# mpkuse/cerebro

Hardware: AMD Instinct MI355X
Metric: loop-queries/sec (ticks of 3 descriptors vs 4096-D x 1M DB) (higher is better)
Workload: dtype f64

## Files before the change

cerebro_amd/csrc/chip_api.hip:

```cpp
#include "chip_internal.h"
#include <cmath>
#include <cstdlib>
#include <cstring>
#include <memory>
#include <new>

using namespace chip;

extern "C" {

const char *chip_strerror(int status)
{
    switch (status) {
        case CHIP_OK: return "ok";
        case CHIP_ERR_INVALID_ARG: return "invalid argument";
        case CHIP_ERR_NO_DEVICE: return "no usable HIP device";
        case CHIP_ERR_HIP: return "HIP runtime error (see chip_last_hip_error)";
        case CHIP_ERR_OOM: return "out of device memory";
        case CHIP_ERR_NOT_F32: return "descriptor value not exactly representable as float32";
        case CHIP_ERR_NONFINITE: return "NaN/Inf in descriptor";
        case CHIP_ERR_RANGE: return "index / length out of range";
        case CHIP_ERR_UNSUPPORTED: return "unsupported configuration";
        case CHIP_ERR_TOO_FEW_POINTS: return "fewer than 20 correspondences";
        case CHIP_ERR_BUSY: return "async slot busy or empty";
// ... 178 lines not shown
    int rc = c->seg_table_dev.alloc(c, kMaxSegs);
    if (rc == CHIP_OK) rc = configure_storage(c, elem);
    if (rc != CHIP_OK) return rc;
    c->stage_bytes = 64ull << 20;
    if (c->stage_bytes < (size_t)c->D * 8 * 64) c->stage_bytes = (size_t)c->D * 8 * 64;
    rc = c->stage_dev.alloc(c, c->stage_bytes);
    if (rc == CHIP_OK) rc = c->flags_dev.alloc(c, 1);
    if (rc == CHIP_OK) rc = c->flags_host.alloc(c, 1);
    if (rc == CHIP_OK) rc = c->norm2_dev.alloc(c, 1);
    if (rc == CHIP_OK) rc = c->norm2_host.alloc(c, 1);
    if (rc != CHIP_OK) return rc;
    CHIP_HIP(c, hipMemset(c->norm2_dev, 0, sizeof(unsigned long long)));
    *c->norm2_host.host() = 0;

    scan_read_knobs(c);
    CHIP_HIP(c, hipStreamCreateWithFlags(&c->s_scan, hipStreamNonBlocking));
    {
        const int ns = c->scan_streams;
        if (ns >= 2) CHIP_HIP(c, hipStreamCreateWithFlags(&c->s_scan2, hipStreamNonBlocking));
        for (int i = 0; i < 2; i++)
            if (ns >= 3 + i) CHIP_HIP(c, hipStreamCreateWithFlags(&c->s_scan_x[i], hipStreamNonBlocking));
    }
    for (int i = 0; i < Ctx::kRing; i++) {
        constexpr size_t kListsPerGroup = 3 * kPrefilterTicks > CHIP_MAX_NQ ? 3 * kPrefilterTicks : CHIP_MAX_NQ;
        static_assert(kPrefilterTicks >= kMultiMaxTicks, "the list buffers are sized for the deepest pass");
        rc = c->partial_dev[i].alloc(c, ((size_t)c->max_grid + 1) * kListsPerGroup * CHIP_MAX_TOPK);
        if (rc != CHIP_OK) return rc;
        CHIP_HIP(c, hipEventCreateWithFlags(&c->ev_scan[i], hipEventDisableTiming));
        CHIP_HIP(c, hipEventCreateWithFlags(&c->ev_merged[i], hipEventDisableTiming));
    }
    rc = c->tickets_dev.alloc(c, Ctx::kRing);
    if (rc != CHIP_OK) return rc;
    CHIP_HIP(c, hipMemset(c->tickets_dev, 0, Ctx::kRing * sizeof(int32_t)));
    c->coalesce_max = env_int("CHIP_TICK_COALESCE", kPrefilterTicks);
    if (c->coalesce_max < 2) c->coalesce_max = 0;
    if (c->coalesce_max > kPrefilterTicks) c->coalesce_max = kPrefilterTicks;
    c->tick_poll = env_int("CHIP_TICK_POLL", 1) != 0;
    resident_read_knobs(c);
    rc = c->seq_all.alloc(c, CHIP_MAX_INFLIGHT);
    if (rc != CHIP_OK) return rc;
    std::memset(c->seq_all.host(), 0, sizeof(unsigned long long) * CHIP_MAX_INFLIGHT);
    rc = c->cert_all.alloc(c, CHIP_MAX_INFLIGHT * 4);
    if (rc != CHIP_OK) return rc;
    std::memset(c->cert_all.host(), 0, sizeof(uint32_t) * CHIP_MAX_INFLIGHT * 4);
    rc = c->topk.alloc(c, (size_t)CHIP_MAX_NQ * CHIP_MAX_TOPK);
    if (rc != CHIP_OK) return rc;
    for (Slot &s : c->slots) {
        CHIP_HIP(c, hipEventCreateWithFlags(&s.done, hipEventDisableTiming));
        rc = s.rec.alloc(c, 1);
        if (rc != CHIP_OK) return rc;
        s.seq_host = c->seq_all.host() + (&s - c->slots);
        s.seq_dev = c->seq_all.dev() + (&s - c->slots);
        s.cert_host = c->cert_all.host() + 4 * (&s - c->slots);
        s.cert_dev = c->cert_all.dev() + 4 * (&s - c->slots);
    }
    if (env_int("CHIP_SCAN_STAMPS", 0)) {
        rc = c->stamps_dev.alloc(c, (size_t)c->max_grid * 16 * 4 + 64);
        if (rc != CHIP_OK) return rc;
        CHIP_HIP(c, hipMemset(c->stamps_dev, 0, ((size_t)c->max_grid * 16 * 4 + 64) * sizeof(unsigned long long)));
    }
    rc = pnp_create(c);
    if (rc != CHIP_OK) return rc;
    c->cap_hint = capacity_hint;
    if (capacity_hint > 0) {
        std::lock_guard<std::mutex> lk(c->append_mu);
        rc = ensure_capacity(c, local_count(c, capacity_hint));
// ... 260 lines not shown
    int fit = scan_multi_max_ticks(c);
    if (c->coalesce_max >= kPrefilterTicks && scan_prefilter_usable(c)) fit = kPrefilterTicks;
    const int t = fit < c->coalesce_max ? fit : c->coalesce_max;
    return t >= 2 ? t : 0;
}

static int coalesce_submit(Ctx *c, int T)
{
    const int b = (int)(c->n_enqueued++ % Ctx::kRing);
    const int K = CHIP_DEFAULT_TOPK;
    const bool prefilter = T == kPrefilterTicks;
    static_assert(kPrefilterTicks > kMultiMaxTicks, "a pass of kPrefilterTicks ticks is the prefilter's");
    PassArgs a{};
    scan_args_db(c, &a);
    a.K = K;
    a.partial = c->partial_dev[b];
    for (int t = 0; t < T; t++) {
        a.k[t] = c->parked[t].k;
        if (a.k[t] > a.n_rows) a.n_rows = a.k[t];
        for (int i = 0; i < 3; i++) a.q[3 * t + i] = c->parked[t].q[i];
    }
    const int grid = scan_multi_grid(c);
    double E = 0.0;
    if (prefilter) {
        std::lock_guard<std::mutex> lk(c->mu);
        E = prefilter_error_bound(c->D, c->row_norm_max);
    }
    if (hipEventQuery(c->ev_merged[b]) != hipSuccess) CHIP_HIP(c, hipStreamWaitEvent(c->s_scan, c->ev_merged[b], 0));
    hipEvent_t e1 = nullptr;
    int rc = c->prof_on ? prof_begin(c, c->s_scan, (double)a.n_rows * c->D * c->elem, &e1) : CHIP_OK;
    if (rc == CHIP_OK) rc = prefilter ? launch_scan_prefilter(c, c->s_scan, a, grid) : launch_scan_multi(c, c->s_scan, a, T, grid);
    if (rc != CHIP_OK) return rc;
    if (e1) CHIP_HIP(c, hipEventRecord(e1, c->s_scan));
    CHIP_HIP(c, hipEventRecord(c->ev_scan[b], c->s_scan));
    c->pass_ev = c->ev_scan[b];
    c->pass_no++;
    CHIP_HIP(c, hipStreamWaitEvent(c->s_query, c->ev_scan[b], 0));
    chip_topk_entry *exact = c->partial_dev[b] + (size_t)kPrefilterTicks * grid * 3 * K;
    if (prefilter) {
        RescoreArgs ra{};
        ra.seg_table = a.seg_table; ra.seg_shift = a.seg_shift; ra.seg_mask = a.seg_mask; ra.D = a.D; ra.K = K;
        ra.in = c->partial_dev[b]; ra.n_lists = grid; ra.wpb = 8;
        ra.E = E;
        ra.out = exact;
        for (int t = 0; t < T; t++) {
            const Ctx::ParkedTick &pt = c->parked[t];
            Slot &s = *pt.slot;
            ra.k[t] = pt.k;
            for (int i = 0; i < 3; i++) { ra.q[3 * t + i] = s.pf_q[i] = pt.q[i]; s.cert_host[i] = 0; }
            ra.cert[t] = s.cert_dev;
            s.prefilter = true; s.pf_k = pt.k; s.pf_p = pt.p;
        }
        rc = launch_rescore(c, c->s_query, ra);
        if (rc != CHIP_OK) return rc;
    }
    for (int t = 0; t < T; t++) {
        const Ctx::ParkedTick &pt = c->parked[t];
        if (prefilter) rc = launch_merge(c, c->s_query, merge_args(exact + (size_t)t * 3 * K, 1, K, nullptr, pt.slot->rec.dev(), pt.l, &pt.p), 3);
        else rc = launch_merge(c, c->s_query, merge_args(c->partial_dev[b] + (size_t)t * grid * 3 * K, grid, K, nullptr, pt.slot->rec.dev(), pt.l, &pt.p), 3);
        if (rc != CHIP_OK) return rc;
        CHIP_HIP(c, hipEventRecord(pt.slot->done, c->s_query));
        pt.slot->wait_ev = pt.slot->done;
        pt.slot->state = SlotState::Event;
        pt.slot->pass_no = c->pass_no;
    }
    CHIP_HIP(c, hipEventRecord(c->ev_merged[b], c->s_query));
    c->coalesce_passes++;
    c->coalesce_ticks += T;
    if (prefilter) { c->prefilter_passes++; c->prefilter_ticks += T; }
    return CHIP_OK;
}

int coalesce_flush(Ctx *c)
{
    const int T = c->n_parked;
    if (T == 0) return CHIP_OK;
    c->n_parked = 0;
    const Ctx::ParkedTick &p0 = c->parked[0];
    int rc;
    if (T == kPrefilterTicks && !scan_prefilter_usable(c)) {
        const Ctx::ParkedTick &pl = c->parked[T - 1];
        rc = coalesce_submit(c, T - 1);
        if (rc == CHIP_OK) rc = tick_submit(c, pl.k, pl.l, &pl.p, pl.q, false, *pl.slot);
    } else {
        rc = T == 1 ? tick_submit(c, p0.k, p0.l, &p0.p, p0.q, false, *p0.slot) : coalesce_submit(c, T);
    }
    for (int t = 0; t < T && rc != CHIP_OK; t++) {
        c->parked[t].slot->state = SlotState::Failed;
        c->parked[t].slot->err = rc;
    }
    return rc;
}

static int tick_enqueue_slot(Ctx *c, int64_t l, const chip_dot_params *p, bool sync_tick, Slot &s)
{
    int32_t status = 0;
    int64_t k = 0;
    const int64_t n_pub = published_rows(c);
    int rc = tick_begin(s, c->xchg ? INT64_MAX : n_pub, &c->last_l, l, p, &status, &k);
// ... 871 lines not shown
```

cerebro_amd/csrc/chip_internal.h:

```cpp
#pragma once
#include <hip/hip_runtime.h>
#include <cstdint>
#include <mutex>
#include <utility>
#include <condition_variable>
#include <vector>
#include "../../include/cerebro_hip.h"

namespace chip {

constexpr int kWave = 64;
constexpr int kMaxSegs = 4096;
constexpr int64_t kSegBytesTarget = 512ll << 20;

struct ScanArgs {
    const void *const *seg_table;
    int32_t seg_shift;
    int64_t seg_mask;
    int64_t n_rows;
    int32_t D;
    int32_t K;
    const void *q[CHIP_MAX_NQ];
    int64_t idx_mul, idx_add;
    chip_topk_entry *partial;
// ... 33 lines not shown
    unsigned long long *exit_host;
    unsigned long long instance;
    unsigned long long lease_ticks;
    uint32_t done;
    uint32_t direct;
};

constexpr int kMultiMaxTicks = 3;
constexpr int kPrefilterTicks = 4;
constexpr int kRescoreCap = 32;
struct PassArgs {
    const void *const *seg_table;
    int32_t seg_shift;
    int64_t seg_mask;
    int64_t n_rows;
    int32_t D;
    int32_t K;
    int64_t k[kPrefilterTicks];
    const void *q[3 * kPrefilterTicks];
    chip_topk_entry *partial;
};
struct RescoreArgs {
    const void *const *seg_table;
    int32_t seg_shift;
    int64_t seg_mask;
    int32_t D;
    int32_t K;
    const chip_topk_entry *in;
    int32_t n_lists;
    int32_t wpb;
    int64_t k[kPrefilterTicks];
    const void *q[3 * kPrefilterTicks];
    double E;
    chip_topk_entry *out;
    uint32_t *cert[kPrefilterTicks];
};

struct MergeArgs {
    const chip_topk_entry *in;
    int32_t n_lists;
    int32_t K;
    chip_topk_entry *out;
    chip_tick_result *result;
    int64_t l;
    int32_t locality;
    double thresh;
};

struct Ctx;

template <class T> class DevBuf {
public:
    DevBuf() = default;
    DevBuf(const DevBuf &) = delete;
    DevBuf &operator=(const DevBuf &) = delete;
    ~DevBuf() { release(); }
    int alloc(Ctx *c, size_t n);
    int reserve(Ctx *c, size_t n);
    void release() { if (p_) (void)hipFree(p_); p_ = nullptr; cap_ = 0; }
    void swap(DevBuf &o) { std::swap(p_, o.p_); std::swap(cap_, o.cap_); }
    T *get() const { return p_; }
    operator T *() const { return p_; }
    size_t capacity() const { return cap_; }
private:
    T *p_ = nullptr;
    size_t cap_ = 0;
};
template <class T> class PinnedBuf {
// ... 38 lines not shown
int project_chunk(Ctx *c, int64_t from, int64_t m);
void project_count_reset(Ctx *c);

struct Vlad {
    DevBuf<char> w;
    DevBuf<float> raw;
    DevBuf<float> x;
    DevBuf<double> a;
    DevBuf<double> part;
    DevBuf<double> vu;
    DevBuf<float> out;
    int32_t C = 0, K = 0, G = 0;
    int32_t last_n = 0;
    int32_t last_maps = 0;
    int bias_count() const { return (K + G + 1) & ~1; }
    double *bias() const { return reinterpret_cast<double *>(w.get()); }
    float *Wt() const { return reinterpret_cast<float *>(w.get() + (size_t)bias_count() * sizeof(double)); }
    float *centres() const { return Wt() + (size_t)(K + G) * C; }
};
int vlad_chunk(Ctx *c, const AppendSrc &src, int64_t from, int64_t m);

int launch_resident(Ctx *c, hipStream_t s, const ResidentArgs &ra, int grid);
int launch_scan(Ctx *c, hipStream_t s, const ScanArgs &a, int nq, int grid);
int launch_merge(Ctx *c, hipStream_t s, const MergeArgs &a, int nq);
int scan_multi_max_ticks(const Ctx *c);
int scan_multi_plan(int D, int elem, int n_ticks, int K, int grid, chip_debug_scan_launch *f);
int scan_multi_grid(const Ctx *c);
int launch_scan_multi(Ctx *c, hipStream_t s, const PassArgs &a, int n_ticks, int grid);
int scan_prefilter_plan(int D, int elem, int K, int grid, chip_debug_scan_launch *f);
bool scan_prefilter_usable(const Ctx *c);
double prefilter_error_bound(int D, double row_norm_max);
int launch_scan_prefilter(Ctx *c, hipStream_t s, const PassArgs &a, int grid);
int launch_rescore(Ctx *c, hipStream_t s, const RescoreArgs &a);
int scan_grid_for(const Ctx *c, int64_t n_rows, int nq, bool q64);
bool scan_q64(const Ctx *c, int nq, bool long_scan);
int scan_rows_form(const Ctx *c, int64_t n_rows, int nq, int grid, bool q64, bool sync_tick = false);
int scan_select(const Ctx *c, const ScanArgs &a, int nq, int grid, chip_debug_scan_launch *f);
int scan_forms_built();
int launch_scores(Ctx *c, hipStream_t s, const ScanArgs &a, double *out_dev);
int launch_store_rows(Ctx *c, hipStream_t s, const void *src, int src_elem, int64_t n, int64_t first_global, uint32_t *flags_dev, bool write_ring,
                      int64_t row_stride = 1);
int launch_synth(Ctx *c, hipStream_t s, int64_t first_global, int64_t n, uint64_t seed,
                 const int64_t *plant_dst_dev, const int64_t *plant_src_dev, const int32_t *plant_kind_dev, int64_t n_plant, int unit);

enum class SlotState : uint8_t {
    Free,
    Immediate,
    Parked,
    Event,
    Poll,
    Resident,
    Failed,
};

struct Slot {
    hipEvent_t done = nullptr;
    hipEvent_t wait_ev = nullptr;
    PinnedBuf<chip_tick_result> rec;
    SlotState state = SlotState::Free;
    int64_t prev_last_l = 0;
    int64_t tick_l = 0;
    unsigned long long *seq_host = nullptr, *seq_dev = nullptr;
    unsigned long long seq_want = 0;
    uint64_t pass_no = 0;
    int32_t err = 0;
    bool prefilter = false;
// ... 61 lines not shown
    int64_t rows_global = 0;
    int64_t rows_local = 0;
    int64_t lossy_rows = 0;
    mutable std::mutex mu;
    std::mutex append_mu;
    mutable std::mutex query_mu;
    std::mutex ring_mu;
    int64_t rows_pending = 0;
    hipEvent_t last_scan_ev[2] = {};
    std::mutex pnp_mu;
    std::mutex icp_mu;

    hipStream_t s_query = nullptr, s_append = nullptr, s_pnp = nullptr;
    bool own_query_stream = true;

    DevBuf<char> stage_dev;
    size_t stage_bytes = 0;
    DevBuf<uint32_t> flags_dev;
    PinnedBuf<uint32_t> flags_host;
    DevBuf<unsigned long long> norm2_dev;
    PinnedBuf<unsigned long long> norm2_host;
    double row_norm_max = 0.0;

    static constexpr int kRing = 64;
    hipStream_t s_scan = nullptr;
    hipStream_t s_scan2 = nullptr;
    hipStream_t s_scan_x[2] = {};
    uint64_t n_same_stream = 0;
    DevBuf<chip_topk_entry> partial_dev[kRing];
    int32_t partial_lists[kRing] = {};
    hipEvent_t ev_scan[kRing] = {};
    hipEvent_t ev_merged[kRing] = {};
    DevBuf<int32_t> tickets_dev;
    PinnedBuf<unsigned long long> seq_all;
    unsigned long long tick_seq = 0;
    bool tick_poll = true;
    bool tick_fused = true;
    Resident res;
    uint64_t n_enqueued = 0;
    int32_t max_grid = 0;
    PinnedBuf<chip_topk_entry> topk;

    DevBuf<char> qvec_dev;
    DevBuf<double> scores_dev;
    DevBuf<unsigned long long> stamps_dev;

    std::vector<char> qconv;
    int64_t cap_hint = 0;
    int32_t group_transport = 0;
    mutable int last_comm = 0;
    int32_t comm_init_abandoned = 0;
    Exchange *xchg = nullptr;
    Group *group = nullptr;
    Ctx *parent = nullptr;
    Slot slots[CHIP_MAX_INFLIGHT];
    int64_t last_l = 0;

    struct ParkedTick { Slot *slot; int64_t k, l; chip_dot_params p; const void *q[3]; };
    int32_t coalesce_max = 4;
    bool coalesce_force = false;
    ParkedTick parked[kPrefilterTicks];
    int32_t n_parked = 0;
    hipEvent_t pass_ev = nullptr;
    uint64_t pass_no = 0;
    int64_t coalesce_passes = 0, coalesce_ticks = 0;
    int64_t prefilter_passes = 0, prefilter_ticks = 0, prefilter_uncertified = 0;
// ... 231 lines not shown
```

cerebro_amd/csrc/kernels.hip:

```cpp
#include "chip_internal.h"
#include "topk_merge.h"
#include <cmath>
#include <type_traits>

namespace chip {

typedef float f32x4 __attribute__((ext_vector_type(4)));
typedef double f64x2 __attribute__((ext_vector_type(2)));

template <typename T> struct Vec16;
template <> struct Vec16<float> { typedef f32x4 type; static constexpr int N = 4; };
template <> struct Vec16<double> { typedef f64x2 type; static constexpr int N = 2; };

template <typename V>
__device__ __forceinline__ const __attribute__((address_space(1))) V *as_global(const V *p)
{
    return (const __attribute__((address_space(1))) V *)p;
}

template <typename V>
__device__ __forceinline__ V stream_load(const V *p)
{
    return __builtin_nontemporal_load(as_global(p));
}
// ... 607 lines not shown
        constexpr int SS = U * NS;
        f32x4 w[SS];
        w[0] = *reinterpret_cast<const f32x4 *>(qv);
        w[1] = *reinterpret_cast<const f32x4 *>(qv + D);
        static_for<U>([&](auto uc) CHIP_INLINE_LAMBDA {
            constexpr int u = uc;
            slot_wait<L - R>();
            static_for<NS>([&](auto qc) CHIP_INLINE_LAMBDA {
                constexpr int q = qc, i = u * NS + q;
                if constexpr (i + 2 < SS) w[i + 2] = *reinterpret_cast<const f32x4 *>(qv + ((i + 2) % NS) * D + ((i + 2) / NS) * 256);
                const f32x2 wl = __builtin_shufflevector(w[i], w[i], 0, 1), wh = __builtin_shufflevector(w[i], w[i], 2, 3);
                static_for<R>([&](auto rr) CHIP_INLINE_LAMBDA { prefilter_fma<pass_row_slot(u, rr)>(acc[rr][q], wl); });
                static_for<R>([&](auto rr) CHIP_INLINE_LAMBDA { prefilter_fma<pass_row_slot(u, rr) + 2>(acc[rr][q], wh); });
                __builtin_amdgcn_sched_barrier(0);
            });
            static_for<NG>([&](auto gc) CHIP_INLINE_LAMBDA {
                constexpr int g = gc, QR = pass_query_slot(NG, u, g);
                slot_wait<L - R - 1 - g>();
                static_for<R>([&](auto rr) CHIP_INLINE_LAMBDA { prefilter_fma_slot<pass_row_slot(u, rr), QR>(acc[rr][NS + g]); });
                static_for<R>([&](auto rr) CHIP_INLINE_LAMBDA { prefilter_fma_slot<pass_row_slot(u, rr) + 2, QR + 2>(acc[rr][NS + g]); });
            });
            slots_issue_kib<u, NG>(voff, row, qg);
        });
    }
};

template <int NG>
__global__ __launch_bounds__(kMultiBlock) __attribute__((amdgpu_num_vgpr(pass_vgpr_base(kPrefilterMaxNG) / 2))) void db_scan_prefilter(PassArgs a)
{
    static_assert(NG <= kPrefilterMaxNG, "the compiler's share is sized for kPrefilterMaxNG query slots per KiB");
    shared_pass<PassF32<NG>>(a);
}

__device__ __forceinline__ void block_best(double &bs, int64_t &bi, double *red_s, int64_t *red_i, int lane, int wave)
{
#pragma unroll
    for (int m = 32; m >= 1; m >>= 1) {
        const double os = __shfl_xor(bs, m, 64);
        const int64_t oi = __shfl_xor(bi, m, 64);
        if (key_gt(os, oi, bs, bi)) { bs = os; bi = oi; }
    }
    __syncthreads();
    if (lane == 0) { red_s[wave] = bs; red_i[wave] = bi; }
    __syncthreads();
    bs = red_s[0]; bi = red_i[0];
#pragma unroll
    for (int w = 1; w < 8; w++)
        if (key_gt(red_s[w], red_i[w], bs, bi)) { bs = red_s[w]; bi = red_i[w]; }
}

__global__ __launch_bounds__(512) void tick_rescore(RescoreArgs a)
{
    constexpr int MAXH = 512 * CHIP_MAX_TOPK / 512;
    __shared__ double red_s[8];
    __shared__ int64_t red_i[8];
    __shared__ chip_topk_entry cand[kRescoreCap];
    __shared__ int n_cand;
    const int tid = threadIdx.x, lane = tid & 63;
    const int wave = __builtin_amdgcn_readfirstlane(tid >> 6);
    const int tick = blockIdx.x / 3, q = blockIdx.x % 3;
    const int K = a.K, n = a.n_lists * K;
    const chip_topk_entry *in = a.in + (int64_t)tick * a.n_lists * 3 * K;
    const int64_t k = a.k[tick];
    if (tid == 0) n_cand = 0;
    double es[MAXH];
    int64_t ei[MAXH];
// ... 17 lines not shown
    block_best(ms, mi, red_s, red_i, lane, wave);
    double gs = INFINITY;
    int64_t gi = INT64_MAX;
    for (int j = 0; j < K; j++) {
        double bs = -INFINITY;
        int64_t bi = -1;
#pragma unroll
        for (int h = 0; h < MAXH; h++)
            if (key_gt(gs, gi, es[h], ei[h]) && key_gt(es[h], ei[h], bs, bi)) { bs = es[h]; bi = ei[h]; }
        block_best(bs, bi, red_s, red_i, lane, wave);
        gs = bs; gi = bi;
    }
    double thr = gs - 2.0 * a.E;
    thr -= fabs(thr) * 0x1p-51;
    const bool ok = mi < 0 || ms < thr;
#pragma unroll
    for (int h = 0; h < MAXH; h++)
        if (ei[h] >= 0 && es[h] >= thr) {
            const int at = atomicAdd(&n_cand, 1);
            if (at < kRescoreCap) { chip_topk_entry t; t.score = es[h]; t.idx = ei[h]; cand[at] = t; }
        }
    __syncthreads();
    const int nc = n_cand < kRescoreCap ? n_cand : kRescoreCap;
    const float *qrow = static_cast<const float *>(a.q[3 * tick + q]);
    for (int j = wave; j < nc; j += 8) {
        const int64_t r = cand[j].idx;
        const float *row[1] = {static_cast<const float *>(a.seg_table[r >> a.seg_shift]) + (r & a.seg_mask) * (int64_t)a.D};
        double acc[1][1];
        rows_dot<float, 1, 4, true, 1, 1>(row, qrow, a.D, lane, acc);
        const double s = butterfly_sum(acc[0][0]);
        if (lane == 0) cand[j].score = s;
    }
    __syncthreads();
    if (wave == 0) {
        static_assert(kRescoreCap <= 64, "one lane per candidate");
        chip_topk_entry *out = a.out + (int64_t)(3 * tick + q) * K;
        chip_topk_entry me;
        me.score = -INFINITY; me.idx = -1;
        if (lane < nc) me = cand[lane];
        int rank = 0;
        for (int j = 0; j < nc; j++) {
            const chip_topk_entry o = cand[j];
            rank += key_gt(o.score, o.idx, me.score, me.idx) ? 1 : 0;
        }
        if (lane < nc && rank < K) out[rank] = me;
        if (lane >= nc && lane < K) out[lane] = me;
        if (lane == 0) a.cert[tick][q] = ok && n_cand <= kRescoreCap ? 1u : 2u;
    }
}

template <int NQ, int NG, bool FULL>
__global__ __launch_bounds__(1024) void db_scan_topk_wide(ScanArgs a)
{
    static_assert(NG >= 1 && NG < NQ, "at least one query staged, at least one read in place");
    extern __shared__ __attribute__((aligned(16))) char smem[];
    double *qs = reinterpret_cast<double *>(smem);
    constexpr int NL = NQ - NG, U = 4, CH = 128;
    const int D = a.D, K = a.K;
    const int tid = threadIdx.x, lane = tid & 63;
    const int wave = __builtin_amdgcn_readfirstlane(tid >> 6);
    const int wpb = blockDim.x >> 6;
    stage_queries<double, NL>(a, qs, tid, blockDim.x);
    __syncthreads();
    const double *qg[NG];
#pragma unroll
    for (int g = 0; g < NG; g++) qg[g] = static_cast<const double *>(a.q[NL + g]);

    double my_s[NQ], thr_s[NQ];
    int64_t my_i[NQ], thr_i[NQ];
#pragma unroll
    for (int q = 0; q < NQ; q++) { my_s[q] = -INFINITY; my_i[q] = -1; thr_s[q] = -INFINITY; thr_i[q] = -1; }
    const int e0 = lane * 2;
    const int64_t tw = (int64_t)gridDim.x * wpb;
    for (int64_t r = (int64_t)blockIdx.x * wpb + wave; r < a.n_rows; r += tw) {
        const double *row = row_base<double>(a, r);
        double acc[NQ];
#pragma unroll
        for (int q = 0; q < NQ; q++) acc[q] = 0.0;
        for (int base = 0; base < D; base += CH * U) {
            f64x2 v[U];
// ... 6 lines not shown
            for (int u = 0; u < U; u++) {
                const int e = base + u * CH + e0;
                if (FULL || e < D) {
#pragma unroll
                    for (int q = 0; q < NQ; q++) {
                        const f64x2 w = q < NL ? *reinterpret_cast<const f64x2 *>(qs + q * D + e)
                                               : *as_global(reinterpret_cast<const f64x2 *>(qg[q < NL ? 0 : q - NL] + e));
                        acc[q] = __builtin_fma(w[0], v[u][0], acc[q]);
                        acc[q] = __builtin_fma(w[1], v[u][1], acc[q]);
                    }
                }
            }
        }
#pragma unroll
        for (int q = 0; q < NQ; q++) acc[q] = butterfly_sum(acc[q]);
        const int64_t gi = r * a.idx_mul + a.idx_add;
#pragma unroll
        for (int q = 0; q < NQ; q++) wave_topk_offer(acc[q], gi, K, lane, my_s[q], my_i[q], thr_s[q], thr_i[q]);
    }
    block_merge_store<NQ>(smem, my_s, my_i, K, lane, wave, wpb, [&](int q) { return a.partial + ((int64_t)blockIdx.x * NQ + q) * K; });
}

__device__ __forceinline__ uint32_t lds_byte_addr(const void *p)
{
    return (uint32_t)(uintptr_t)(const __attribute__((address_space(3))) void *)p;
}
__device__ __forceinline__ void glds16_q(const void *gsrc_lane, uint32_t lds_base_wave_uniform)
{
    unsigned keep;
    asm volatile("s_mov_b32 %0, m0\n\ts_mov_b32 m0, %2\n\ts_nop 0\n\tglobal_load_lds_dwordx4 %1, off\n\ts_mov_b32 m0, %0"
                 : "=&s"(keep)
                 : "v"(gsrc_lane), "s"(lds_base_wave_uniform)
                 : "memory");
}

__device__ __forceinline__ void store_entry_agent(chip_topk_entry *p, double s, int64_t i)
{
    __hip_atomic_store(reinterpret_cast<unsigned long long *>(&p->score), (unsigned long long)__double_as_longlong(s), __ATOMIC_RELAXED, __HIP_MEMORY_SCOPE_AGENT);
    __hip_atomic_store(reinterpret_cast<unsigned long long *>(&p->idx), (unsigned long long)i, __ATOMIC_RELAXED, __HIP_MEMORY_SCOPE_AGENT);
}
__device__ __forceinline__ chip_topk_entry load_entry_agent(const chip_topk_entry *p)
{
    chip_topk_entry e;
    e.score = __longlong_as_double((long long)__hip_atomic_load(reinterpret_cast<const unsigned long long *>(&p->score), __ATOMIC_RELAXED, __HIP_MEMORY_SCOPE_AGENT));
    e.idx = (int64_t)__hip_atomic_load(reinterpret_cast<const unsigned long long *>(&p->idx), __ATOMIC_RELAXED, __HIP_MEMORY_SCOPE_AGENT);
    return e;
}

template <int NQ>
__device__ __forceinline__ void block_merge_lists(const ScanArgs &a, const chip_topk_entry *lists, int K, int lane, int wave, int wpb, bool coherent = false)
{
    __syncthreads();
    for (int q = wave; q < NQ; q += wpb) {
        const int ncand = wpb * K;
        double cs[4];
        int64_t ci[4];
#pragma unroll
        for (int h = 0; h < 4; h++) {
            const int c = lane + 64 * h;
            if (c < ncand) {
                const chip_topk_entry t = lists[((c / K) * NQ + q) * CHIP_MAX_TOPK + (c % K)];
                cs[h] = t.score;
                ci[h] = t.idx;
            } else { cs[h] = -INFINITY; ci[h] = -1; }
        }
        chip_topk_entry *outp = a.partial + ((int64_t)blockIdx.x * NQ + q) * K;
        for (int j = 0; j < K; j++) {
            double bs = cs[0];
            int64_t bi = ci[0];
#pragma unroll
            for (int h = 1; h < 4; h++)
                if (key_gt(cs[h], ci[h], bs, bi)) { bs = cs[h]; bi = ci[h]; }
#pragma unroll
            for (int m = 32; m >= 1; m >>= 1) {
                const double os = __shfl_xor(bs, m, 64);
                const int64_t oi = __shfl_xor(bi, m, 64);
                if (key_gt(os, oi, bs, bi)) { bs = os; bi = oi; }
            }
#pragma unroll
// ... 846 lines not shown
    }
}

int launch_scores(Ctx *c, hipStream_t s, const ScanArgs &a, double *out_dev)
{
    const size_t lds = (size_t)c->D * c->elem;
    int64_t grid = (a.n_rows + 7) / 8;
    if (grid > (int64_t)c->n_cus * 4) grid = (int64_t)c->n_cus * 4;
    if (grid < 1) grid = 1;
    const int chunk = 64 * (16 / c->elem) * 4;
    const bool full = a.D % chunk == 0;
    if (c->elem == 8) {
        if (lds > 65536) {
            CHIP_HIP(c, hipFuncSetAttribute(reinterpret_cast<const void *>(db_scan_scores<double, true>), hipFuncAttributeMaxDynamicSharedMemorySize, (int)lds));
            CHIP_HIP(c, hipFuncSetAttribute(reinterpret_cast<const void *>(db_scan_scores<double, false>), hipFuncAttributeMaxDynamicSharedMemorySize, (int)lds));
        }
        if (full) hipLaunchKernelGGL((db_scan_scores<double, true>), dim3((int)grid), dim3(512), lds, s, a, out_dev);
        else hipLaunchKernelGGL((db_scan_scores<double, false>), dim3((int)grid), dim3(512), lds, s, a, out_dev);
    } else {
        if (full) hipLaunchKernelGGL((db_scan_scores<float, true>), dim3((int)grid), dim3(512), lds, s, a, out_dev);
        else hipLaunchKernelGGL((db_scan_scores<float, false>), dim3((int)grid), dim3(512), lds, s, a, out_dev);
    }
    CHIP_HIP(c, hipGetLastError());
    return CHIP_OK;
}

template <int NQ>
__global__ __launch_bounds__(512) void topk_merge(MergeArgs a)
{
    __shared__ __attribute__((aligned(16))) char smem[kMergeSmem];
    merge_sorted_lists<NQ>(a.in, a.n_lists, NQ, 0, a.K, a.out, a.result, a.l, a.locality, a.thresh, smem);
}

int launch_merge(Ctx *c, hipStream_t s, const MergeArgs &a, int nq)
{
    if (a.n_lists > 512) return CHIP_ERR_UNSUPPORTED;
    switch (nq) {
        case 1: hipLaunchKernelGGL(topk_merge<1>, dim3(1), dim3(512), 0, s, a); break;
        case 2: hipLaunchKernelGGL(topk_merge<2>, dim3(1), dim3(512), 0, s, a); break;
        case 3: hipLaunchKernelGGL(topk_merge<3>, dim3(1), dim3(512), 0, s, a); break;
        case 4: hipLaunchKernelGGL(topk_merge<4>, dim3(1), dim3(512), 0, s, a); break;
        default: return CHIP_ERR_UNSUPPORTED;
    }
    CHIP_HIP(c, hipGetLastError());
    return CHIP_OK;
}

struct StoreArgs {
    void *const *seg_table;
    int32_t seg_shift;
    int64_t seg_mask;
    void *ring;
    int32_t D;
    int32_t rank, nranks;
    int64_t first_global;
    int64_t row_stride;
    int64_t n;
    int64_t ring_from;
    uint32_t *flags;
};

template <typename T>
__device__ __forceinline__ void store_row4(const StoreArgs &a, int64_t g, int e, const T (&v)[4])
{
    typedef typename Vec16<T>::type V;
    constexpr int N = Vec16<T>::N;
// ... 242 lines not shown
```

cerebro_amd/csrc/topk_merge.h:

```cpp
#pragma once
#include "chip_internal.h"
#include <cmath>

namespace chip {

__device__ __forceinline__ bool key_gt(double s, int64_t i, double s2, int64_t i2)
{
    return s > s2 || (s == s2 && i > i2);
}

constexpr int kMergeSmem = 28 * 1024;
constexpr int64_t kFailedShardIdx = -2;
constexpr int kSurvCap = CHIP_MAX_TOPK * CHIP_MAX_TOPK;

__device__ __forceinline__ double readlane_f64(double v, int j)
{
    const long long b = __double_as_longlong(v);
    const int lo = __builtin_amdgcn_readlane((int)(b & 0xffffffffll), j);
    const int hi = __builtin_amdgcn_readlane((int)(b >> 32), j);
    return __longlong_as_double(((long long)hi << 32) | (unsigned int)lo);
}
__device__ __forceinline__ int64_t readlane_i64(int64_t v, int j)
{
    const int lo = __builtin_amdgcn_readlane((int)(v & 0xffffffffll), j);
    const int hi = __builtin_amdgcn_readlane((int)(v >> 32), j);
    return ((int64_t)hi << 32) | (unsigned int)lo;
}

__device__ __forceinline__ unsigned long long okey(double s)
{
    const unsigned long long b0 = (unsigned long long)__double_as_longlong(s);
    const unsigned long long b = b0 == 0x8000000000000000ull ? 0ull : b0;
    return (b >> 63) ? ~b : (b | 0x8000000000000000ull);
}

__device__ __forceinline__ int wave_rank(double s, int64_t i, bool valid)
{
    const unsigned kh = (unsigned)(okey(s) >> 32);
    int rank = 0, eq = 0;
#pragma unroll 16
    for (int j = 0; j < 64; j++) {
        const unsigned o = (unsigned)__builtin_amdgcn_readlane((int)kh, j);
        rank += o > kh ? 1 : 0;
        eq += o == kh ? 1 : 0;
    }
    if (__ballot(valid && eq > 1) == 0ull) return rank;
    rank = 0;
#pragma unroll 8
    for (int j = 0; j < 64; j++) rank += key_gt(readlane_f64(s, j), readlane_i64(i, j), s, i) ? 1 : 0;
    return rank;
}

__device__ __forceinline__ void wave_rank2(const double s[2], const int64_t i[2], int &r0, int &r1)
{
    const unsigned k0 = (unsigned)(okey(s[0]) >> 32), k1 = (unsigned)(okey(s[1]) >> 32);
    int e0 = 0, e1 = 0;
    r0 = r1 = 0;
#pragma unroll 16
    for (int j = 0; j < 64; j++) {
        const unsigned a = (unsigned)__builtin_amdgcn_readlane((int)k0, j), b = (unsigned)__builtin_amdgcn_readlane((int)k1, j);
        r0 += (a > k0 ? 1 : 0) + (b > k0 ? 1 : 0);
        e0 += (a == k0 ? 1 : 0) + (b == k0 ? 1 : 0);
        r1 += (a > k1 ? 1 : 0) + (b > k1 ? 1 : 0);
        e1 += (a == k1 ? 1 : 0) + (b == k1 ? 1 : 0);
    }
    if (__ballot((i[0] >= 0 && e0 > 1) || (i[1] >= 0 && e1 > 1)) == 0ull) return;
    r0 = r1 = 0;
#pragma unroll 8
    for (int j = 0; j < 64; j++) {
        const double a0 = readlane_f64(s[0], j), a1 = readlane_f64(s[1], j);
        const int64_t b0 = readlane_i64(i[0], j), b1 = readlane_i64(i[1], j);
        r0 += (key_gt(a0, b0, s[0], i[0]) ? 1 : 0) + (key_gt(a1, b1, s[0], i[0]) ? 1 : 0);
        r1 += (key_gt(a0, b0, s[1], i[1]) ? 1 : 0) + (key_gt(a1, b1, s[1], i[1]) ? 1 : 0);
    }
}

template <int NQ>
__device__ __forceinline__ void merge_sorted_lists(const chip_topk_entry *in, int n_lists, int list_stride, int q_off, int K, chip_topk_entry *out,
                                                   chip_tick_result *result, int64_t l, int locality, double thresh, char *smem)
{
    chip_topk_entry *candA = reinterpret_cast<chip_topk_entry *>(smem);
    chip_topk_entry *surv = candA + CHIP_MAX_NQ * 8 * CHIP_MAX_TOPK;
    chip_topk_entry *T1s = surv + CHIP_MAX_NQ * kSurvCap;
    chip_topk_entry *tops = T1s + CHIP_MAX_NQ;
    int *cnt = reinterpret_cast<int *>(tops + CHIP_MAX_NQ);
    int *failed = cnt + CHIP_MAX_NQ;
    const int t = threadIdx.x;
    const int lane = t & 63, w = t >> 6, nw = blockDim.x >> 6;

    double hs[NQ];
    int64_t hi[NQ];
#pragma unroll
    for (int q = 0; q < NQ; q++) {
        if (t < n_lists) { const chip_topk_entry x = in[((int64_t)t * list_stride + q_off + q) * K]; hs[q] = x.score; hi[q] = x.idx; }
        else { hs[q] = -INFINITY; hi[q] = -1; }
    }
    if (t < NQ) cnt[t] = 0;
    if (t == NQ) *failed = 0;
#pragma unroll
    for (int q = 0; q < NQ; q++) {
        const bool valid = hi[q] >= 0;
        const int rank = wave_rank(hs[q], hi[q], valid);
        const int nvalid = __popcll(__ballot(valid));
        chip_topk_entry *dst = candA + (q * 8 + w) * CHIP_MAX_TOPK;
        if (valid && rank < K) { dst[rank].score = hs[q]; dst[rank].idx = hi[q]; }
        if (lane < K && lane >= nvalid) { dst[lane].score = -INFINITY; dst[lane].idx = -1; }
    }
// ... 26 lines not shown
            double es[CHIP_MAX_TOPK];
            int64_t ei[CHIP_MAX_TOPK];
            es[0] = hs[q]; ei[0] = hi[q];
#pragma unroll
            for (int j = 1; j < CHIP_MAX_TOPK; j++) {
                if (j < K) { const chip_topk_entry x = in[((int64_t)t * list_stride + q_off + q) * K + j]; es[j] = x.score; ei[j] = x.idx; }
                else { es[j] = -INFINITY; ei[j] = -1; }
            }
            int c = 1;
#pragma unroll
            for (int j = 1; j < CHIP_MAX_TOPK; j++)
                if (c == j && ei[j] >= 0 && !key_gt(ts, ti, es[j], ei[j])) c = j + 1;
            const int base = atomicAdd(&cnt[q], c);
#pragma unroll
            for (int j = 0; j < CHIP_MAX_TOPK; j++)
                if (j < c && base + j < kSurvCap) { surv[q * kSurvCap + base + j].score = es[j]; surv[q * kSurvCap + base + j].idx = ei[j]; }
        }
    }
    __syncthreads();
    if (w < NQ) {
        const int q = w;
        int n = cnt[q];
        if (n > kSurvCap) n = kSurvCap;
        double cs[4];
        int64_t ci[4];
        int rk[4];
#pragma unroll
        for (int h = 0; h < 4; h++) {
            const int c = lane + 64 * h;
            if (c < n) { cs[h] = surv[q * kSurvCap + c].score; ci[h] = surv[q * kSurvCap + c].idx; }
            else { cs[h] = -INFINITY; ci[h] = -1; }
            rk[h] = 0;
        }
        for (int j = 0; j < n; j++) {
            const chip_topk_entry x = surv[q * kSurvCap + j];
#pragma unroll
            for (int h = 0; h < 4; h++) rk[h] += key_gt(x.score, x.idx, cs[h], ci[h]) ? 1 : 0;
        }
#pragma unroll
        for (int h = 0; h < 4; h++) {
            if (ci[h] >= 0 && rk[h] < K) {
                if (out) { out[q * K + rk[h]].score = cs[h]; out[q * K + rk[h]].idx = ci[h]; }
                if (rk[h] == 0) { tops[q].score = cs[h]; tops[q].idx = ci[h]; }
            }
        }
        if (lane < K && lane >= n) {
            if (out) { out[q * K + lane].score = -INFINITY; out[q * K + lane].idx = -1; }
            if (lane == 0) { tops[q].score = -INFINITY; tops[q].idx = -1; }
        }
    }
    __syncthreads();
    if (out != nullptr && t == 0 && *failed) out[0].idx = kFailedShardIdx;
    if (result != nullptr && t == 0) {
        chip_tick_result res;
        res.status = *failed ? CHIP_TICK_FAILED : CHIP_TICK_SCANNED;
        res.found = 0;
        res.idx_curr = -1;
        res.idx_prev = -1;
        res.score = 0.0;
        for (int q = 0; q < 3; q++) {
            res.argmax[q] = q < NQ ? tops[q].idx : -1;
            res.maxv[q] = q < NQ ? tops[q].score : -INFINITY;
        }
        if (NQ >= 3 && res.argmax[0] >= 0 && res.argmax[1] >= 0 && res.argmax[2] >= 0) {
            int64_t d1 = res.argmax[0] - res.argmax[1];
            int64_t d2 = res.argmax[0] - res.argmax[2];
            if (d1 < 0) d1 = -d1;
            if (d2 < 0) d2 = -d2;
            if (d1 < locality && d2 < locality && res.maxv[0] > thresh) {
                res.found = 1;
                res.idx_curr = l - 1;
                res.idx_prev = res.argmax[0];
                res.score = res.maxv[0];
            }
        }
        *result = res;
    }
}


}
```

Baseline: 1204.

## Fuse per-tick merge into rescore/pass-finish kernels on the scan stream

In the prefilter path, the rescore kernel now writes only each query's best entry. The last-arriving block per tick, detected with an agent-scope atomic counter, computes the tick decision and writes the result record directly, so the T per-tick merge launches are no longer needed. The non-prefilter path replaces the T merge launches with a single pass_finish kernel that has one block per tick. All post-scan work moves onto the scan stream, and slots wait on a single ev_merged event, which removes the cross-stream event hops. Some rank-loop unroll factors are also reduced, likely to cut register pressure. The cost is extra atomic coordination logic, and the rescore no longer emits a full top-K list.

Measured after the change: 1203. Within noise of the previous version (-0.1%).

```diff
diff --git a/cerebro_amd/csrc/chip_api.hip b/cerebro_amd/csrc/chip_api.hip
--- a/cerebro_amd/csrc/chip_api.hip
+++ b/cerebro_amd/csrc/chip_api.hip
@@ -234,6 +234,9 @@
     rc = c->tickets_dev.alloc(c, Ctx::kRing);
     if (rc != CHIP_OK) return rc;
     CHIP_HIP(c, hipMemset(c->tickets_dev, 0, Ctx::kRing * sizeof(int32_t)));
+    rc = c->arrive_dev.alloc(c, (size_t)Ctx::kRing * kPrefilterTicks);
+    if (rc != CHIP_OK) return rc;
+    CHIP_HIP(c, hipMemset(c->arrive_dev, 0, (size_t)Ctx::kRing * kPrefilterTicks * sizeof(int32_t)));
     c->coalesce_max = env_int("CHIP_TICK_COALESCE", kPrefilterTicks);
     if (c->coalesce_max < 2) c->coalesce_max = 0;
     if (c->coalesce_max > kPrefilterTicks) c->coalesce_max = kPrefilterTicks;
@@ -560,39 +563,42 @@
     if (rc == CHIP_OK) rc = prefilter ? launch_scan_prefilter(c, c->s_scan, a, grid) : launch_scan_multi(c, c->s_scan, a, T, grid);
     if (rc != CHIP_OK) return rc;
     if (e1) CHIP_HIP(c, hipEventRecord(e1, c->s_scan));
-    CHIP_HIP(c, hipEventRecord(c->ev_scan[b], c->s_scan));
-    c->pass_ev = c->ev_scan[b];
-    c->pass_no++;
-    CHIP_HIP(c, hipStreamWaitEvent(c->s_query, c->ev_scan[b], 0));
-    chip_topk_entry *exact = c->partial_dev[b] + (size_t)kPrefilterTicks * grid * 3 * K;
     if (prefilter) {
         RescoreArgs ra{};
         ra.seg_table = a.seg_table; ra.seg_shift = a.seg_shift; ra.seg_mask = a.seg_mask; ra.D = a.D; ra.K = K;
         ra.in = c->partial_dev[b]; ra.n_lists = grid; ra.wpb = 8;
         ra.E = E;
-        ra.out = exact;
+        ra.best = c->partial_dev[b] + (size_t)kPrefilterTicks * grid * 3 * K;
+        ra.arrive = c->arrive_dev + (size_t)b * kPrefilterTicks;
         for (int t = 0; t < T; t++) {
             const Ctx::ParkedTick &pt = c->parked[t];
             Slot &s = *pt.slot;
             ra.k[t] = pt.k;
             for (int i = 0; i < 3; i++) { ra.q[3 * t + i] = s.pf_q[i] = pt.q[i]; s.cert_host[i] = 0; }
             ra.cert[t] = s.cert_dev;
+            ra.rec[t] = s.rec.dev(); ra.l[t] = pt.l; ra.locality[t] = pt.p.locality; ra.thresh[t] = pt.p.thresh;
             s.prefilter = true; s.pf_k = pt.k; s.pf_p = pt.p;
         }
-        rc = launch_rescore(c, c->s_query, ra);
-        if (rc != CHIP_OK) return rc;
-    }
+        rc = launch_rescore(c, c->s_scan, ra);
+    } else {
+        PassFinishArgs fa{};
+        fa.in = c->partial_dev[b]; fa.n_lists = grid; fa.K = K;
+        for (int t = 0; t < T; t++) {
+            const Ctx::ParkedTick &pt = c->parked[t];
+            fa.rec[t] = pt.slot->rec.dev(); fa.l[t] = pt.l; fa.locality[t] = pt.p.locality; fa.thresh[t] = pt.p.thresh;
+        }
+        rc = launch_pass_finish(c, c->s_scan, fa, T);
+    }
+    if (rc != CHIP_OK) return rc;
+    CHIP_HIP(c, hipEventRecord(c->ev_merged[b], c->s_scan));
+    c->pass_ev = c->ev_merged[b];
+    c->pass_no++;
     for (int t = 0; t < T; t++) {
-        const Ctx::ParkedTick &pt = c->parked[t];
-        if (prefilter) rc = launch_merge(c, c->s_query, merge_args(exact + (size_t)t * 3 * K, 1, K, nullptr, pt.slot->rec.dev(), pt.l, &pt.p), 3);
-        else rc = launch_merge(c, c->s_query, merge_args(c->partial_dev[b] + (size_t)t * grid * 3 * K, grid, K, nullptr, pt.slot->rec.dev(), pt.l, &pt.p), 3);
-        if (rc != CHIP_OK) return rc;
-        CHIP_HIP(c, hipEventRecord(pt.slot->done, c->s_query));
-        pt.slot->wait_ev = pt.slot->done;
-        pt.slot->state = SlotState::Event;
-        pt.slot->pass_no = c->pass_no;
-    }
-    CHIP_HIP(c, hipEventRecord(c->ev_merged[b], c->s_query));
+        Slot &s = *c->parked[t].slot;
+        s.wait_ev = c->ev_merged[b];
+        s.state = SlotState::Event;
+        s.pass_no = c->pass_no;
+    }
     c->coalesce_passes++;
     c->coalesce_ticks += T;
     if (prefilter) { c->prefilter_passes++; c->prefilter_ticks += T; }
diff --git a/cerebro_amd/csrc/chip_internal.h b/cerebro_amd/csrc/chip_internal.h
--- a/cerebro_amd/csrc/chip_internal.h
+++ b/cerebro_amd/csrc/chip_internal.h
@@ -89,8 +89,22 @@
     int64_t k[kPrefilterTicks];
     const void *q[3 * kPrefilterTicks];
     double E;
-    chip_topk_entry *out;
+    chip_topk_entry *best;
     uint32_t *cert[kPrefilterTicks];
+    int32_t *arrive;
+    chip_tick_result *rec[kPrefilterTicks];
+    int64_t l[kPrefilterTicks];
+    int32_t locality[kPrefilterTicks];
+    double thresh[kPrefilterTicks];
+};
+struct PassFinishArgs {
+    const chip_topk_entry *in;
+    int32_t n_lists;
+    int32_t K;
+    chip_tick_result *rec[kMultiMaxTicks];
+    int64_t l[kMultiMaxTicks];
+    int32_t locality[kMultiMaxTicks];
+    double thresh[kMultiMaxTicks];
 };
 
 struct MergeArgs {
@@ -195,6 +209,7 @@
 double prefilter_error_bound(int D, double row_norm_max);
 int launch_scan_prefilter(Ctx *c, hipStream_t s, const PassArgs &a, int grid);
 int launch_rescore(Ctx *c, hipStream_t s, const RescoreArgs &a);
+int launch_pass_finish(Ctx *c, hipStream_t s, const PassFinishArgs &a, int n_ticks);
 int scan_grid_for(const Ctx *c, int64_t n_rows, int nq, bool q64);
 bool scan_q64(const Ctx *c, int nq, bool long_scan);
 int scan_rows_form(const Ctx *c, int64_t n_rows, int nq, int grid, bool q64, bool sync_tick = false);
@@ -322,6 +337,7 @@
     hipEvent_t ev_scan[kRing] = {};
     hipEvent_t ev_merged[kRing] = {};
     DevBuf<int32_t> tickets_dev;
+    DevBuf<int32_t> arrive_dev;
     PinnedBuf<unsigned long long> seq_all;
     unsigned long long tick_seq = 0;
     bool tick_poll = true;
diff --git a/cerebro_amd/csrc/kernels.hip b/cerebro_amd/csrc/kernels.hip
--- a/cerebro_amd/csrc/kernels.hip
+++ b/cerebro_amd/csrc/kernels.hip
@@ -663,6 +663,19 @@
     shared_pass<PassF32<NG>>(a);
 }
 
+__device__ __forceinline__ void store_entry_agent(chip_topk_entry *p, double s, int64_t i)
+{
+    __hip_atomic_store(reinterpret_cast<unsigned long long *>(&p->score), (unsigned long long)__double_as_longlong(s), __ATOMIC_RELAXED, __HIP_MEMORY_SCOPE_AGENT);
+    __hip_atomic_store(reinterpret_cast<unsigned long long *>(&p->idx), (unsigned long long)i, __ATOMIC_RELAXED, __HIP_MEMORY_SCOPE_AGENT);
+}
+__device__ __forceinline__ chip_topk_entry load_entry_agent(const chip_topk_entry *p)
+{
+    chip_topk_entry e;
+    e.score = __longlong_as_double((long long)__hip_atomic_load(reinterpret_cast<const unsigned long long *>(&p->score), __ATOMIC_RELAXED, __HIP_MEMORY_SCOPE_AGENT));
+    e.idx = (int64_t)__hip_atomic_load(reinterpret_cast<const unsigned long long *>(&p->idx), __ATOMIC_RELAXED, __HIP_MEMORY_SCOPE_AGENT);
+    return e;
+}
+
 __device__ __forceinline__ void block_best(double &bs, int64_t &bi, double *red_s, int64_t *red_i, int lane, int wave)
 {
 #pragma unroll
@@ -746,20 +759,28 @@
         if (lane == 0) cand[j].score = s;
     }
     __syncthreads();
-    if (wave == 0) {
-        static_assert(kRescoreCap <= 64, "one lane per candidate");
-        chip_topk_entry *out = a.out + (int64_t)(3 * tick + q) * K;
-        chip_topk_entry me;
-        me.score = -INFINITY; me.idx = -1;
-        if (lane < nc) me = cand[lane];
-        int rank = 0;
+    if (tid == 0) {
+        double bs = -INFINITY;
+        int64_t bi = -1;
         for (int j = 0; j < nc; j++) {
             const chip_topk_entry o = cand[j];
-            rank += key_gt(o.score, o.idx, me.score, me.idx) ? 1 : 0;
-        }
-        if (lane < nc && rank < K) out[rank] = me;
-        if (lane >= nc && lane < K) out[lane] = me;
-        if (lane == 0) a.cert[tick][q] = ok && n_cand <= kRescoreCap ? 1u : 2u;
+            if (key_gt(o.score, o.idx, bs, bi)) { bs = o.score; bi = o.idx; }
+        }
+        a.cert[tick][q] = ok && n_cand <= kRescoreCap ? 1u : 2u;
+        store_entry_agent(a.best + 3 * tick + q, bs, bi);
+        __threadfence();
+        if (__hip_atomic_fetch_add(a.arrive + tick, 1, __ATOMIC_RELAXED, __HIP_MEMORY_SCOPE_AGENT) == 2) {
+            __builtin_amdgcn_fence(__ATOMIC_ACQUIRE, "agent");
+            chip_topk_entry top[3];
+#pragma unroll
+            for (int i = 0; i < 3; i++) {
+                const chip_topk_entry o = load_entry_agent(a.best + 3 * tick + i);
+                top[i].score = i == q ? bs : o.score;
+                top[i].idx = i == q ? bi : o.idx;
+            }
+            *a.rec[tick] = tick_decide(top, true, false, a.l[tick], a.locality[tick], a.thresh[tick]);
+            __hip_atomic_store(a.arrive + tick, 0, __ATOMIC_RELAXED, __HIP_MEMORY_SCOPE_AGENT);
+        }
     }
 }
 
@@ -832,19 +853,6 @@
                  : "=&s"(keep)
                  : "v"(gsrc_lane), "s"(lds_base_wave_uniform)
                  : "memory");
-}
-
-__device__ __forceinline__ void store_entry_agent(chip_topk_entry *p, double s, int64_t i)
-{
-    __hip_atomic_store(reinterpret_cast<unsigned long long *>(&p->score), (unsigned long long)__double_as_longlong(s), __ATOMIC_RELAXED, __HIP_MEMORY_SCOPE_AGENT);
-    __hip_atomic_store(reinterpret_cast<unsigned long long *>(&p->idx), (unsigned long long)i, __ATOMIC_RELAXED, __HIP_MEMORY_SCOPE_AGENT);
-}
-__device__ __forceinline__ chip_topk_entry load_entry_agent(const chip_topk_entry *p)
-{
-    chip_topk_entry e;
-    e.score = __longlong_as_double((long long)__hip_atomic_load(reinterpret_cast<const unsigned long long *>(&p->score), __ATOMIC_RELAXED, __HIP_MEMORY_SCOPE_AGENT));
-    e.idx = (int64_t)__hip_atomic_load(reinterpret_cast<const unsigned long long *>(&p->idx), __ATOMIC_RELAXED, __HIP_MEMORY_SCOPE_AGENT);
-    return e;
 }
 
 template <int NQ>
@@ -1757,6 +1765,21 @@
     merge_sorted_lists<NQ>(a.in, a.n_lists, NQ, 0, a.K, a.out, a.result, a.l, a.locality, a.thresh, smem);
 }
 
+__global__ __launch_bounds__(512) void pass_finish(PassFinishArgs a)
+{
+    __shared__ __attribute__((aligned(16))) char smem[kMergeSmem];
+    const int t = blockIdx.x;
+    merge_sorted_lists<3>(a.in + (int64_t)t * a.n_lists * 3 * a.K, a.n_lists, 3, 0, a.K, nullptr, a.rec[t], a.l[t], a.locality[t], a.thresh[t], smem);
+}
+
+int launch_pass_finish(Ctx *c, hipStream_t s, const PassFinishArgs &a, int n_ticks)
+{
+    if (a.n_lists > 512 || n_ticks < 1 || n_ticks > kMultiMaxTicks) return CHIP_ERR_UNSUPPORTED;
+    hipLaunchKernelGGL(pass_finish, dim3(n_ticks), dim3(512), 0, s, a);
+    CHIP_HIP(c, hipGetLastError());
+    return CHIP_OK;
+}
+
 int launch_merge(Ctx *c, hipStream_t s, const MergeArgs &a, int nq)
 {
     if (a.n_lists > 512) return CHIP_ERR_UNSUPPORTED;
diff --git a/cerebro_amd/csrc/topk_merge.h b/cerebro_amd/csrc/topk_merge.h
--- a/cerebro_amd/csrc/topk_merge.h
+++ b/cerebro_amd/csrc/topk_merge.h
@@ -46,7 +46,7 @@
     }
     if (__ballot(valid && eq > 1) == 0ull) return rank;
     rank = 0;
-#pragma unroll 8
+#pragma unroll 2
     for (int j = 0; j < 64; j++) rank += key_gt(readlane_f64(s, j), readlane_i64(i, j), s, i) ? 1 : 0;
     return rank;
 }
@@ -66,13 +66,40 @@
     }
     if (__ballot((i[0] >= 0 && e0 > 1) || (i[1] >= 0 && e1 > 1)) == 0ull) return;
     r0 = r1 = 0;
-#pragma unroll 8
+#pragma unroll 1
     for (int j = 0; j < 64; j++) {
         const double a0 = readlane_f64(s[0], j), a1 = readlane_f64(s[1], j);
         const int64_t b0 = readlane_i64(i[0], j), b1 = readlane_i64(i[1], j);
         r0 += (key_gt(a0, b0, s[0], i[0]) ? 1 : 0) + (key_gt(a1, b1, s[0], i[0]) ? 1 : 0);
         r1 += (key_gt(a0, b0, s[1], i[1]) ? 1 : 0) + (key_gt(a1, b1, s[1], i[1]) ? 1 : 0);
     }
+}
+
+__device__ __forceinline__ chip_tick_result tick_decide(const chip_topk_entry (&top)[3], bool three, bool failed, int64_t l, int locality, double thresh)
+{
+    chip_tick_result res;
+    res.status = failed ? CHIP_TICK_FAILED : CHIP_TICK_SCANNED;
+    res.found = 0;
+    res.idx_curr = -1;
+    res.idx_prev = -1;
+    res.score = 0.0;
+    for (int q = 0; q < 3; q++) {
+        res.argmax[q] = top[q].idx;
+        res.maxv[q] = top[q].score;
+    }
+    if (three && res.argmax[0] >= 0 && res.argmax[1] >= 0 && res.argmax[2] >= 0) {
+        int64_t d1 = res.argmax[0] - res.argmax[1];
+        int64_t d2 = res.argmax[0] - res.argmax[2];
+        if (d1 < 0) d1 = -d1;
+        if (d2 < 0) d2 = -d2;
+        if (d1 < locality && d2 < locality && res.maxv[0] > thresh) {
+            res.found = 1;
+            res.idx_curr = l - 1;
+            res.idx_prev = res.argmax[0];
+            res.score = res.maxv[0];
+        }
+    }
+    return res;
 }
 
 template <int NQ>
@@ -165,6 +192,7 @@
             else { cs[h] = -INFINITY; ci[h] = -1; }
             rk[h] = 0;
         }
+#pragma unroll 2
         for (int j = 0; j < n; j++) {
             const chip_topk_entry x = surv[q * kSurvCap + j];
 #pragma unroll
@@ -185,31 +213,14 @@
     __syncthreads();
     if (out != nullptr && t == 0 && *failed) out[0].idx = kFailedShardIdx;
     if (result != nullptr && t == 0) {
-        chip_tick_result res;
-        res.status = *failed ? CHIP_TICK_FAILED : CHIP_TICK_SCANNED;
-        res.found = 0;
-        res.idx_curr = -1;
-        res.idx_prev = -1;
-        res.score = 0.0;
+        chip_topk_entry top[3];
         for (int q = 0; q < 3; q++) {
-            res.argmax[q] = q < NQ ? tops[q].idx : -1;
-            res.maxv[q] = q < NQ ? tops[q].score : -INFINITY;
-        }
-        if (NQ >= 3 && res.argmax[0] >= 0 && res.argmax[1] >= 0 && res.argmax[2] >= 0) {
-            int64_t d1 = res.argmax[0] - res.argmax[1];
-            int64_t d2 = res.argmax[0] - res.argmax[2];
-            if (d1 < 0) d1 = -d1;
-            if (d2 < 0) d2 = -d2;
-            if (d1 < locality && d2 < locality && res.maxv[0] > thresh) {
-                res.found = 1;
-                res.idx_curr = l - 1;
-                res.idx_prev = res.argmax[0];
-                res.score = res.maxv[0];
-            }
-        }
-        *result = res;
-    }
-}
-
-
-}
+            top[q].idx = q < NQ ? tops[q].idx : -1;
+            top[q].score = q < NQ ? tops[q].score : -INFINITY;
+        }
+        *result = tick_decide(top, NQ >= 3, *failed != 0, l, locality, thresh);
+    }
+}
+
+
+}
```
